# sipposip/pr-disagg-radar-gan

Measured on AMD Instinct MI355X. Metric: cWGAN-GP train samples/sec, 24x16x16 tiles, bs=256, higher is better.
Workload: dtype f32; 1 GPU; ndomain=16, 24h, bs=256 fp32, 1 critic step + 1 gen step (BASELINE configs[1]); batch_per_gpu=256, global_batch=256, n_critic=1, parallelism=dp1, world=1, rccl_ranks_seen=1, weights=random init (RandomNormal 0.02 / glorot_uniform), dropout 0.25 active

## Files before the change

### include/rdgan.h

```cpp
#ifndef RDGAN_H
#define RDGAN_H
#include <stdint.h>
#ifdef __cplusplus
extern "C" {
#endif

typedef struct rdgan_handle rdgan_handle;

#define RDGAN_LATENT_DIM 100
#define RDGAN_NHOURS 24
#define RDGAN_LOSS_SLOTS 8

int rdgan_create(rdgan_handle** out, int ndomain, int n_cond_channels, int max_batch);
void rdgan_destroy(rdgan_handle* h);
const char* rdgan_last_error(const rdgan_handle* h);
long rdgan_gen_param_count(const rdgan_handle* h);
long rdgan_critic_param_count(const rdgan_handle* h);
long rdgan_workspace_bytes(const rdgan_handle* h);

int rdgan_gen_forward(rdgan_handle* h, const float* gen_params, const float* z, const float* cond,
                      float* out, int B, void* stream);

int rdgan_check_numerics(rdgan_handle* h, void* stream);

// ... 128 lines not shown
int rdgan_op_upconv_slab_t16(const float* x, const float* w, const float* bias, float* y, float* rinv, float* dbg, int B, int H, int W,
                             void* stream);
int rdgan_op_upconv2_slab16(const float* x, const float* w, const float* bias, float* y, float* rinv, int B, void* stream);
int rdgan_op_upconv_wgrad_slab16(const float* x, const float* dy, float* dWc, int B, void* stream);
int rdgan_op_d2_fwd_slab16(const float* x, const float* w, const float* bias, float* y, int B, uint64_t seed, void* stream);
int rdgan_op_d2_wgrad_slab16(const float* x, const float* dy, float* dW, int B, void* stream);
int rdgan_op_d2_wgrad_slab_t16(const float* x, const float* dy, float* dW, int B, int OH, int OW, void* stream);
int rdgan_op_d3_wgrad_slab16(const float* x, const float* dy, float* dW, int B, void* stream);
int rdgan_op_d2_dgrad_slab16(const float* gy, const float* w, const float* aux, float* gx, int B, int use_drop, void* stream);
int rdgan_op_d2_dgrad_slab_t16(const float* gy, const float* w, const float* aux, float* gx, int B, int OH, int OW, int use_drop,
                               void* stream);
int rdgan_op_pixelnorm_lrelu(const float* y, float* h, float* rinv, long npix, int C, void* stream);
int rdgan_op_pixelnorm_lrelu_bwd(const float* gh, const float* h, const float* rinv, float* dy,
                                 long npix, int C, void* stream);
int rdgan_debug_activation(rdgan_handle* h, int which, float* out, long n, void* stream);
int rdgan_op_rng(uint64_t seed, uint32_t stream_id, float* mask_out, float* uniform_out, long n,
                 void* stream);

#ifdef __cplusplus
}
#endif
#endif
```

### pr_disagg_radar_gan_amd/_lib.py

```python
import ctypes
import os

_HERE = os.path.dirname(os.path.abspath(__file__))
LIB_PATH = os.path.join(_HERE, "librdgan_hip.so")

c_f32p = ctypes.c_void_p
c_stream = ctypes.c_void_p

class LaunchStat(ctypes.Structure):
    _fields_ = [("plan", ctypes.c_int), ("kind", ctypes.c_int), ("batch", ctypes.c_int), ("launches", ctypes.c_int),
                ("gflop", ctypes.c_double), ("ms", ctypes.c_double), ("name", ctypes.c_char * 48), ("kernel", ctypes.c_char * 48)]


SIGNATURES = {
    "rdgan_create": (ctypes.c_int, [ctypes.POINTER(ctypes.c_void_p), ctypes.c_int, ctypes.c_int, ctypes.c_int]),
    "rdgan_destroy": (None, [ctypes.c_void_p]),
    "rdgan_last_error": (ctypes.c_char_p, [ctypes.c_void_p]),
    "rdgan_gen_param_count": (ctypes.c_long, [ctypes.c_void_p]),
    "rdgan_critic_param_count": (ctypes.c_long, [ctypes.c_void_p]),
    "rdgan_workspace_bytes": (ctypes.c_long, [ctypes.c_void_p]),
    "rdgan_gen_forward": (ctypes.c_int, [ctypes.c_void_p, c_f32p, c_f32p, c_f32p, c_f32p, ctypes.c_int, c_stream]),
    "rdgan_check_numerics": (ctypes.c_int, [ctypes.c_void_p, c_stream]),
    "rdgan_critic_forward": (ctypes.c_int, [ctypes.c_void_p, c_f32p, c_f32p, c_f32p, c_f32p, ctypes.c_int,
                                            ctypes.c_uint64, c_stream]),
# ... 71 lines not shown
    "rdgan_op_fastd_wgrad": (ctypes.c_int, [c_f32p, c_f32p, c_f32p] + [ctypes.c_int] * 8 + [c_stream]),
    "rdgan_op_g9_wgrad": (ctypes.c_int, [c_f32p, c_f32p, c_f32p] + [ctypes.c_int] * 4 + [c_stream]),
    "rdgan_op_upconv_slab16": (ctypes.c_int, [c_f32p] * 6 + [ctypes.c_int, c_stream]),
    "rdgan_op_upconv_slab_t16": (ctypes.c_int, [c_f32p] * 6 + [ctypes.c_int] * 3 + [c_stream]),
    "rdgan_op_upconv2_slab16": (ctypes.c_int, [c_f32p] * 5 + [ctypes.c_int, c_stream]),
    "rdgan_op_upconv_wgrad_slab16": (ctypes.c_int, [c_f32p] * 3 + [ctypes.c_int, c_stream]),
    "rdgan_op_d2_fwd_slab16": (ctypes.c_int, [c_f32p] * 4 + [ctypes.c_int, ctypes.c_uint64, c_stream]),
    "rdgan_op_d3_wgrad_slab16": (ctypes.c_int, [c_f32p] * 3 + [ctypes.c_int, c_stream]),
    "rdgan_op_d2_wgrad_slab16": (ctypes.c_int, [c_f32p] * 3 + [ctypes.c_int, c_stream]),
    "rdgan_op_d2_wgrad_slab_t16": (ctypes.c_int, [c_f32p] * 3 + [ctypes.c_int] * 3 + [c_stream]),
    "rdgan_op_d2_dgrad_slab16": (ctypes.c_int, [c_f32p] * 4 + [ctypes.c_int, ctypes.c_int, c_stream]),
    "rdgan_op_d2_dgrad_slab_t16": (ctypes.c_int, [c_f32p] * 4 + [ctypes.c_int] * 4 + [c_stream]),
    "rdgan_op_pixelnorm_lrelu": (ctypes.c_int, [c_f32p, c_f32p, c_f32p, ctypes.c_long, ctypes.c_int, c_stream]),
    "rdgan_op_pixelnorm_lrelu_bwd": (ctypes.c_int, [c_f32p, c_f32p, c_f32p, c_f32p, ctypes.c_long, ctypes.c_int, c_stream]),
    "rdgan_debug_activation": (ctypes.c_int, [ctypes.c_void_p, ctypes.c_int, c_f32p, ctypes.c_long, c_stream]),
    "rdgan_op_rng": (ctypes.c_int, [ctypes.c_uint64, ctypes.c_uint32, c_f32p, c_f32p, ctypes.c_long, c_stream]),
}

TAG_GCONV_FWD, TAG_GCONV_DGRAD, TAG_GCONV_WGRAD, TAG_CRITIC_GEMM, TAG_ELEMENTWISE, TAG_GCONV3_FWD = range(6)

_lib = None


class RdganError(RuntimeError):
    pass


class NumericsError(RdganError, ArithmeticError):
    """tf.debugging.check_numerics behind the generator's softmax (reference T:349-350) fired: NaN/Inf in the output."""

# ... 27 lines not shown
```

### pr_disagg_radar_gan_amd/csrc/rdgan_api.hip

```cpp
#include <hip/hip_runtime.h>
#include <stdio.h>
#include <string.h>
#include <math.h>
#include <string>
#include <vector>
#include <algorithm>
#include <unordered_set>

#include "../../include/rdgan.h"
#include "rdgan_plan.h"
#include "rdgan_hostplan.h"
#include "rdgan_rng.h"
#include "rdgan_gemm.hip.h"
#include "rdgan_gemm_ws.hip.h"
#include "rdgan_gemm_ws16.hip.h"
#include "rdgan_gemm_f16.hip.h"
#include "rdgan_upconv16.hip.h"
#include "rdgan_upconv16b.hip.h"
#include "rdgan_upconv16t.hip.h"
#include "rdgan_elem.hip.h"
#include "rdgan_data.hip.h"
#include "rdgan_edge.hip.h"
#include "rdgan_d2slab16.hip.h"
#include "rdgan_d2fwd16.hip.h"
// ... 40 lines not shown
  int wgrad_wide = 0;
  int conv_f16 = 1;
  void* bW3I;
  int upconv_slab = 1;
  void* bW3T = nullptr;
  int upconv_slab_t = 1;
  void* bW2I = nullptr;
  int upconv2_slab = 1;
  int g9_fused = 1;
  void* bW9I;
  void* bW2S;
  int d3_wgrad_slab = 1;
  int d2_wgrad_slab = 1;
  int upwgrad_slab = 1;
  int d1_dgrad_fused = 1;
  int d1_wgrad16 = 1;
  void* bW2F = nullptr;
  int d2_fwd_slab = 0;
  unsigned char* g1bits = nullptr;
  int dense16 = 1;
  int dense_skinny = 1;
  void* xcat16 = nullptr;
  void* bW0 = nullptr;
  int g9_bwd_mfma = 1;
  int d1_fwd_sample = 1;
  int wgrad_boxes = 1;
  int border_boxes = 1;
  int d2_gate_bits = 1;
  int d2_slab = 1;
  int a16 = 0;
// ... 622 lines not shown
  const rd_bf16_t* y16 = (const rd_bf16_t*)y; rd_bf16_t* h16 = (rd_bf16_t*)hout;
  if (a16) {
    if (C == 256) hipLaunchKernelGGL((k_pixelnorm_lrelu_fwd<64, rd_bf16_t>), grid, dim3(256), 0, st, y16, h16, rinv, npix);
    else if (C == 128) hipLaunchKernelGGL((k_pixelnorm_lrelu_fwd<32, rd_bf16_t>), grid, dim3(256), 0, st, y16, h16, rinv, npix);
    else if (C == 64) hipLaunchKernelGGL((k_pixelnorm_lrelu_fwd<16, rd_bf16_t>), grid, dim3(256), 0, st, y16, h16, rinv, npix);
    else return bad_arg(h, "pixelnorm: C must be 64/128/256");
  }
  else if (C == 256) hipLaunchKernelGGL(k_pixelnorm_lrelu_fwd<64>, grid, dim3(256), 0, st, y, hout, rinv, npix);
  else if (C == 128) hipLaunchKernelGGL(k_pixelnorm_lrelu_fwd<32>, grid, dim3(256), 0, st, y, hout, rinv, npix);
  else if (C == 64) hipLaunchKernelGGL(k_pixelnorm_lrelu_fwd<16>, grid, dim3(256), 0, st, y, hout, rinv, npix);
  else return bad_arg(h, "pixelnorm: C must be 64/128/256");
  RD_CHECK(h, hipGetLastError());
  return 0;
}
static int launch_pn_bwd(rdgan_handle* h, const float* g, const float* hh, const float* rinv, float* dy, long npix, int C,
                         int pool, int D, int H, int W, hipStream_t st, bool a16 = false) {
  long threads = npix * (C / 4);
  dim3 grid((unsigned)((threads + 255) / 256));
#define RD_PNB(LP, PO) hipLaunchKernelGGL((k_pn_lrelu_bwd<LP, PO>), grid, dim3(256), 0, st, g, hh, rinv, dy, npix, D, H, W)
#define RD_PNB16(LP) hipLaunchKernelGGL((k_pn_lrelu_bwd<LP, 0, rd_bf16_t>), grid, dim3(256), 0, st, (const rd_bf16_t*)g, \
                                        (const rd_bf16_t*)hh, rinv, (rd_bf16_t*)dy, npix, D, H, W)
  if (a16) {
    if (pool) return bad_arg(h, "pixelnorm bwd: the bf16 storage mode needs the collapsed form");
    if (C == 256) RD_PNB16(64); else if (C == 128) RD_PNB16(32); else if (C == 64) RD_PNB16(16);
    else return bad_arg(h, "pixelnorm bwd: C must be 64/128/256");
  }
  else if (C == 256) { if (pool) RD_PNB(64, 1); else RD_PNB(64, 0); }
  else if (C == 128) { if (pool) RD_PNB(32, 1); else RD_PNB(32, 0); }
  else if (C == 64) { if (pool) RD_PNB(16, 1); else RD_PNB(16, 0); }
  else return bad_arg(h, "pixelnorm bwd: C must be 64/128/256");
#undef RD_PNB
#undef RD_PNB16
  RD_CHECK(h, hipGetLastError());
  return 0;
}

static int launch_pn_bwd_pairs(rdgan_handle* h, const float* g, const float* hh, const float* rinv, float* dy, float* gS,
                               long npair, long HW, int C, hipStream_t st, bool a16 = false) {
  long threads = npair * (C / 4);
  dim3 grid((unsigned)((threads + 255) / 256));
#define RD_PNP16(LP) hipLaunchKernelGGL((k_pn_lrelu_bwd_pairs<LP, rd_bf16_t>), grid, dim3(256), 0, st, (const rd_bf16_t*)g, \
                                        (const rd_bf16_t*)hh, rinv, (rd_bf16_t*)dy, (rd_bf16_t*)gS, npair, HW)
  if (a16) {
    if (C == 256) RD_PNP16(64); else if (C == 128) RD_PNP16(32); else if (C == 64) RD_PNP16(16);
    else return bad_arg(h, "pixelnorm bwd: C must be 64/128/256");
  }
  else if (C == 256) hipLaunchKernelGGL(k_pn_lrelu_bwd_pairs<64>, grid, dim3(256), 0, st, g, hh, rinv, dy, gS, npair, HW);
  else if (C == 128) hipLaunchKernelGGL(k_pn_lrelu_bwd_pairs<32>, grid, dim3(256), 0, st, g, hh, rinv, dy, gS, npair, HW);
  else if (C == 64) hipLaunchKernelGGL(k_pn_lrelu_bwd_pairs<16>, grid, dim3(256), 0, st, g, hh, rinv, dy, gS, npair, HW);
  else return bad_arg(h, "pixelnorm bwd: C must be 64/128/256");
#undef RD_PNP16
  RD_CHECK(h, hipGetLastError());
  return 0;
}


extern "C" int rdgan_create(rdgan_handle** out, int ndomain, int n_cond_channels, int max_batch) {
  if (!out) return -2;
  *out = nullptr;
  if (!rd_geometry_ok(ndomain, n_cond_channels, max_batch)) return -2;
  rdgan_handle* h = new rdgan_handle();
  rd_geometry(h, ndomain, n_cond_channels, max_batch);
  const int nd = ndomain;
  const int* gch = h->gch; const int* dch = h->dch;
// ... 195 lines not shown
  if (!strcmp(name, "resident")) { h->resident = value ? 1 : 0; return 0; }
  if (!strcmp(name, "upconv_slab")) { h->upconv_slab = value ? 1 : 0; return 0; }
  if (!strcmp(name, "upconv_slab_t")) { h->upconv_slab_t = value ? 1 : 0; return 0; }
  if (!strcmp(name, "upconv2_slab")) { h->upconv2_slab = value ? 1 : 0; return 0; }
  if (!strcmp(name, "g9_fused")) { h->g9_fused = value ? 1 : 0; return 0; }
  if (!strcmp(name, "d1_fwd_sample")) { h->d1_fwd_sample = value ? 1 : 0; return 0; }
  if (!strcmp(name, "g9_bwd_mfma")) { h->g9_bwd_mfma = value ? 1 : 0; return 0; }
  if (!strcmp(name, "dense16")) { h->dense16 = value ? 1 : 0; return 0; }
  if (!strcmp(name, "dense_skinny")) { h->dense_skinny = value ? 1 : 0; return 0; }
  if (!strcmp(name, "wgrad_boxes")) { h->wgrad_boxes = value ? 1 : 0; return 0; }
  if (!strcmp(name, "border_boxes")) { h->border_boxes = value < 0 ? 0 : (value > 2 ? 2 : value); return 0; }
  if (!strcmp(name, "d3_wgrad_slab")) { h->d3_wgrad_slab = value ? 1 : 0; return 0; }
  if (!strcmp(name, "d2_wgrad_slab")) { h->d2_wgrad_slab = value ? 1 : 0; return 0; }
  if (!strcmp(name, "upwgrad_slab")) { h->upwgrad_slab = value ? 1 : 0; return 0; }
  if (!strcmp(name, "d1_dgrad_fused")) { h->d1_dgrad_fused = value ? 1 : 0; return 0; }
  if (!strcmp(name, "d1_wgrad16")) { h->d1_wgrad16 = value ? 1 : 0; return 0; }
  if (!strcmp(name, "wgrad_wide")) { h->wgrad_wide = value ? 1 : 0; return 0; }
  if (!strcmp(name, "conv_f16")) {
    if (value < 0 || value > 2) return bad_arg(h, "conv_f16: 0, 1 or 2 (2: regardless of the launch size)");
    h->conv_f16 = value; h->ccache_ver = 0; h->gcache_ver = 0; return 0;
  }
  if (!strcmp(name, "d2_fwd_slab")) { h->d2_fwd_slab = value ? 1 : 0; h->ccache_ver = 0; return 0; }
  if (!strcmp(name, "d2_gate_bits")) { h->d2_gate_bits = value ? 1 : 0; return 0; }
  if (!strcmp(name, "d2_slab")) { h->d2_slab = value ? 1 : 0; h->ccache_ver = 0; return 0; }
  if (!strcmp(name, "dense_wgrad_slices")) { h->dense_slices = value; return 0; }
  if (!strcmp(name, "keep_gates")) {
    h->keep_gates = value ? 1 : 0;
    h->gate_keep_B = 0;
    for (int l = 1; l <= 4 && h->keep_gates; ++l)
      if (!h->gate_keep[l]) RD_CHECK(h, hipMalloc(&h->gate_keep[l], (size_t)h->MB * h->dL[l] * h->dch[l] * sizeof(float)));
// ... 655 lines not shown
      const int one = PL_D2B;
      RD_TRY(launch_d2_dgrad_slab_t(h, {one, plan_flops(h->plans[one], NBt), RDGAN_TAG_CRITIC_GEMM}, h->du[2], h->bW2S, h->dh[1], h->du[1], NBt,
                                    h->ddim[2][1], h->ddim[2][2], use_drop, gbits, st));
      continue;
    }
    if (a16)
      RD_TRY(launch_conv16(h, h->plans[pl], h->d_plans + pl, NBt, h->du[l], h->bWB[l], h->du[l - 1], ep, st, RDGAN_TAG_CRITIC_GEMM,
                           h->conv_f16 ? h->fWB[l] : nullptr));
    else
    RD_TRY(launch_conv(h, h->plans[pl], h->d_plans + pl, NBt, h->du[l], h->DWT[l], h->dch[l - 1], h->du[l - 1], ep, st,
                       RDGAN_TAG_CRITIC_GEMM));
  }
  return 0;
}

static int critic_input_grad(rdgan_handle* h, const float* dp, const float* u1, int B, hipStream_t st) {
  if (h->a16 && h->d1_dgrad_fused && h->nd == 16 && d1_gemm_ok(h)) {
    ProfScope ps(h, RDGAN_TAG_CRITIC_GEMM, st);
    LaunchScope ls(h, PL_D1B, RD_KIND_CONV, B, 2.0 * B * h->dL[1] * 27 * 64, st);
    RD_KNAME(h, "k_d1_dgrad_sample16<bf16>");
    h->flops_acc += 2.0 * B * h->dL[1] * 27 * 64;
    RD_TRY(ensure_lds(h, (const void*)k_d1_dgrad_sample16, RD_D1DG_LDS));
    hipLaunchKernelGGL(k_d1_dgrad_sample16, dim3((unsigned)std::min(B, 512)), dim3(256), RD_D1DG_LDS, st, (const rd_bf16_t*)u1,
                       dp + h->doff[0], h->g0, B);
    RD_CHECK(h, hipGetLastError());
    return 0;
  }
  if (h->a16 && h->d1_dgrad_fused && h->nd > 16 && h->nd % 16 == 0 && d1_gemm_ok(h)) {
    ProfScope ps(h, RDGAN_TAG_CRITIC_GEMM, st);
    LaunchScope ls(h, PL_D1B, RD_KIND_CONV, B, 2.0 * B * h->dL[1] * 27 * 64, st);
    RD_KNAME(h, "k_d1_dgrad_tile16<bf16>");
// ... 2 lines not shown
    const long items = (long)B * (h->nd / 16) * (h->nd / 8);
    hipLaunchKernelGGL(k_d1_dgrad_tile16, dim3((unsigned)std::min<long>(items, 1024)), dim3(256), RD_D1DT_LDS, st, (const rd_bf16_t*)u1,
                       dp + h->doff[0], h->g0, B, h->nd);
    RD_CHECK(h, hipGetLastError());
    return 0;
  }
  if (h->a16)
    RD_TRY(launch_conv16(h, h->plans[PL_D1B], h->d_plans + PL_D1B, B, u1, h->bW1B, h->P1, epi_make(RD_EPI_PLAIN), st,
                         RDGAN_TAG_CRITIC_GEMM));
  else
  RD_TRY(launch_conv(h, h->plans[PL_D1B], h->d_plans + PL_D1B, B, u1, h->W1T, h->ldp1, h->P1, epi_make(RD_EPI_PLAIN), st,
                     RDGAN_TAG_CRITIC_GEMM));
  ProfScope ps(h, RDGAN_TAG_ELEMENTWISE, st);
  hipLaunchKernelGGL(k_d1_col2im, dim3(ew_blocks((long)B * h->dL[0])), dim3(256), 0, st, h->P1, h->g0, B, h->ddim[0][0],
                     h->ddim[0][1], h->ddim[0][2], h->ddim[1][0], h->ddim[1][1], h->ddim[1][2], h->Cin, h->ldp1);
  RD_CHECK(h, hipGetLastError());
  return 0;
}

extern "C" int rdgan_critic_forward(rdgan_handle* h, const float* critic_params, const float* sample, const float* cond,
                                    float* out, int B, uint64_t seed, void* stream) {
  if (!h || !critic_params || !sample || !cond || !out) return bad_arg(h, "critic_forward: null pointer");
  if (B < 1 || B > h->NB) return bad_arg(h, "critic_forward: B outside [1, 3*max_batch]");
  hipStream_t st = (hipStream_t)stream;
  RD_TRY(ahead_drain(h, st));
  h->gate_keep_B = 0;
  RD_TRY(a16_check(h));
  if (h->a16) RD_TRY(prep_critic_weights(h, critic_params, st));
  else if (h->CP != h->Cin && !(h->cver_in != 0 && critic_params == h->ccache_ptr && h->cver_in == h->ccache_ver)) {
    hipLaunchKernelGGL(k_pad_w1, dim3(27), dim3(256), 0, st, critic_params + h->doff[0], h->W1P, h->Cin, h->CP);
// ... 36 lines not shown
  const bool a16 = h->a16 != 0;
  {
    ProfScope ps(h, RDGAN_TAG_ELEMENTWISE, st);
    launch_build_critic_input(h, x_real, h->fake, cond, B, 0, rd_make_key(seed, RD_STREAM_ALPHA), (uint32_t)h->sample_offset, st);
  }
  if (gen_z && fwd_ahead_on(h)) RD_TRY(ahead_issue(h, gp, gen_z, gen_cond, gen_B, st));
  RD_TRY(critic_forward_impl(h, dp, NBt, seed, st));
  RD_TRY(critic_dgrad_chain(h, dp, NBt, B, 0, seed, st));
  {
    hipStream_t cs = side_fork(h, st);
    for (int l = 1; l <= 4; ++l) {
      if (l == 1 && d1_gemm_ok(h) && d1_wgrad16_on(h)) continue;
      RD_TRY(launch_colsum(h, h->du[l], (long)2 * B * h->dL[l], h->dch[l], grad + h->doff[2 * (l - 1) + 1], cs, h->a16 != 0));
    }
  }
  RD_TRY(critic_input_grad(h, dp, act_off(h, h->du[1], (long)2 * B * h->dL[1] * 64), B, st));
  float* cin_hat = h->cin + (long)2 * B * h->dL[0] * h->CP;
  {
    ProfScope ps(h, RDGAN_TAG_ELEMENTWISE, st);
    const int per = (int)h->dL[0];
    const int S = std::max(1, std::min({(1024 + B - 1) / B, per / 4096, 64}));
    if (S > 1) hipLaunchKernelGGL(k_gp_norm_part, dim3(B * S), dim3(256), 0, st, h->g0, h->gp_part, per, S);
    hipLaunchKernelGGL(k_gp_norm_r0, dim3(B * S), dim3(256), 0, st, h->g0, cin_hat, h->gpv, per, B, RD_GP_WEIGHT, h->CP, S, h->gp_part);
  }
  h->gate_keep_B = 0;
  if (h->keep_gates) {
    for (int l = 1; l <= 4; ++l) {
      const long third = (long)2 * B * h->dL[l] * h->dch[l];
      RD_CHECK(h, hipMemcpyAsync(h->gate_keep[l], act_off(h, h->dh[l], third), (size_t)(third / 2) * (a16 ? 2 : 4),
                                 hipMemcpyDeviceToDevice, st));
    }
    h->gate_keep_B = B;
  }
  {
    const float* in = cin_hat;
    for (int l = 1; l <= 4; ++l) {
      int pl = l == 1 ? PL_D1F : critic_fwd_plan(h, l, B);
      long third = (long)2 * B * h->dL[l] * h->dch[l];
      float* dst = act_off(h, h->dh[l], third);
// ... 117 lines not shown
    RD_TRY(launch_wgrad(h, h->plans[PL_G9B], h->d_plans + PL_G9B, B, h->P9, h->h3, grad + h->goff[8], h->wpartial,
                        h->wpartial_cap, st, RDGAN_TAG_GCONV_WGRAD));
    RD_TRY(launch_conv(h, h->plans[PL_G9B], h->d_plans + PL_G9B, B, h->P9, gp + h->goff[8], 64, h->gh3,
                       epi_make(RD_EPI_PLAIN), st, RDGAN_TAG_GCONV_DGRAD));
  }
  {
    hipStream_t cs = side_fork(h, st);
    RD_TRY(launch_colsum(h, h->dl, npix3 / 64, 64, h->g9b_tmp, cs));
    RD_TRY(launch_colsum(h, h->g9b_tmp, 64, 1, grad + h->goff[9], cs));
  }
  float* hs[4] = {h->h0, h->h1, h->h2, h->h3};
  float* rs[4] = {nullptr, h->r1, h->r2, h->r3};
  float* dys[4] = {nullptr, h->dy1, h->dy2, h->gh3};
  float* gups[4] = {nullptr, h->gup1, h->gup2, h->gup3};
  const int col = h->collapse;
  if (col) {
    RdSliceMap map;
    collapsed_dgrad_slice_map(map.src);
    for (int l = 1; l <= 3; ++l) {
      if (gen_block_fast(h, l, fast_bwd_on(h))) continue;
      if (gen_block_fast(h, l, fast_fwd_on(h)))
        hipLaunchKernelGGL(k_collapse_weights, dim3(ew_blocks(16L * h->gch[l - 1] * h->gch[l])), dim3(256), 0, st,
                           gp + h->goff[2 * l], h->GWC[l], h->gch[l - 1] * h->gch[l]);
      if (a16) continue;
      hipLaunchKernelGGL(k_transpose_map, dim3((h->gch[l] + 31) / 32, (h->gch[l - 1] + 31) / 32, 64), dim3(256), 0, st,
                         h->GWC[l], h->GWD[l], h->gch[l - 1], h->gch[l], map);
    }
  }
  for (int l = 3; l >= 1; --l) {
    const bool fast = gen_block_fast(h, l, fast_bwd_on(h));
// ... 5 lines not shown
        const int nunits = B * (RDGAN_NHOURS / 2 / PP);
        RD_TRY(ensure_lds(h, (const void*)k_g9_bwd_mfma16, lds9));
        hipLaunchKernelGGL(k_g9_bwd_mfma16, dim3((unsigned)std::min(nunits, PP > 1 ? 768 : 1536)), dim3(256), lds9, st, h->dl, gp + h->goff[8],
                           (const rd_bf16_t*)hs[3], rs[3], (rd_bf16_t*)dys[3], nunits, RDGAN_NHOURS, nd, nd, PP);
      } else
      if (a16) hipLaunchKernelGGL(k_g9_bwd_pairs<rd_bf16_t>, dim3(B * (RDGAN_NHOURS / 2)), dim3(256), g9_lds, st, h->dl, gp + h->goff[8],
                                  (const rd_bf16_t*)hs[3], rs[3], (rd_bf16_t*)dys[3], fast ? (rd_bf16_t*)h->fgS : (rd_bf16_t*)nullptr,
                                  RDGAN_NHOURS, nd, nd);
      else hipLaunchKernelGGL(k_g9_bwd_pairs<float>, dim3(B * (RDGAN_NHOURS / 2)), dim3(256), g9_lds, st, h->dl, gp + h->goff[8],
                              (const float*)hs[3], rs[3], dys[3], fast ? h->fgS : (float*)nullptr, RDGAN_NHOURS, nd, nd);
      RD_CHECK(h, hipGetLastError());
    } else if (fast) {
      ProfScope ps(h, RDGAN_TAG_ELEMENTWISE, st);
      const long HW = (long)h->gdim[l][1] * h->gdim[l][2];
      RD_TRY(launch_pn_bwd_pairs(h, l == 3 ? h->gh3 : gups[l + 1], hs[l], rs[l], dys[l], h->fgS, (long)B * h->gdim[l - 1][0] * HW,
                                 HW, h->gch[l], st, a16));
    } else {
      ProfScope ps(h, RDGAN_TAG_ELEMENTWISE, st);
      if (l == 3) RD_TRY(launch_pn_bwd(h, h->gh3, hs[3], rs[3], dys[3], npix3, 64, 0, 0, 0, 0, st, a16));
      else RD_TRY(launch_pn_bwd(h, gups[l + 1], hs[l], rs[l], dys[l], (long)B * h->gpix[l], h->gch[l], col ? 0 : 1,
                                h->gdim[l][0], h->gdim[l][1], h->gdim[l][2], st, a16));
    }
    const long cc = (long)h->gch[l - 1] * h->gch[l];
    if (fast) {
      const int* sd = h->gdim[l - 1];
      const int D = sd[0];
      const long P = (long)sd[1] * sd[2] * h->gch[l - 1];
      RdWeightMap wm;
      fastd_weight_map(wm);
      {
        ProfScope ps(h, RDGAN_TAG_ELEMENTWISE, st);
        if (!gen_block_fast(h, l, fast_fwd_on(h))) {
          const dim3 dg(ew_blocks((long)B * (D + 1) * P / 4));
          if (a16) hipLaunchKernelGGL(k_diff_d<rd_bf16_t>, dg, dim3(256), 0, st, (const rd_bf16_t*)hs[l - 1], (rd_bf16_t*)h->fE[l], B, D, P);
          else
          hipLaunchKernelGGL(k_diff_d<float>, dg, dim3(256), 0, st, (const float*)hs[l - 1],
                             h->fE[l], B, D, P);
// ... 32 lines not shown
        }
        RD_TRY(launch_conv16(h, h->plans[pbs], h->d_plans + pbs, B, h->fgS, h->bUT, gups[l], eb, st, RDGAN_TAG_GCONV_DGRAD));
        RD_TRY(launch_conv16(h, h->plans[pbe], h->d_plans + pbe, B, dys[l], h->bUT, h->fdE, eb, st, RDGAN_TAG_GCONV_DGRAD));
      } else {
        {
          RdSliceMap map;
          fastd_dgrad_slice_map(map.src);
          hipLaunchKernelGGL(k_transpose_map, dim3((h->gch[l] + 31) / 32, (h->gch[l - 1] + 31) / 32, 48), dim3(256), 0, st, h->fU[l],
                             h->fUT, h->gch[l - 1], h->gch[l], map);
        }
        RD_TRY(launch_conv(h, h->plans[pbs], h->d_plans + pbs, B, h->fgS, h->fUT, h->gch[l - 1], gups[l], eb, st,
                           RDGAN_TAG_GCONV_DGRAD));
        RD_TRY(launch_conv(h, h->plans[pbe], h->d_plans + pbe, B, dys[l], h->fUT, h->gch[l - 1], h->fdE, eb, st,
                           RDGAN_TAG_GCONV_DGRAD));
      }
      {
        ProfScope ps(h, RDGAN_TAG_ELEMENTWISE, st);
        const dim3 cg(ew_blocks((long)B * D * P / 4));
        if (a16) hipLaunchKernelGGL(k_combine_dx<rd_bf16_t>, cg, dim3(256), 0, st, (rd_bf16_t*)gups[l], (const rd_bf16_t*)h->fdE, B, D, P);
        else hipLaunchKernelGGL(k_combine_dx<float>, cg, dim3(256), 0, st, gups[l], (const float*)h->fdE, B, D, P);
      }
    } else if (col) {
      int plf = PL_G1FC + l - 1, plb = gen_box_plan(h, PL_G1BC + l - 1, PL_G1BCX + l - 1, B);
      const int plfx = PL_G1FCX + l - 1;
      const bool wbox = h->wgrad_boxes && h->border_boxes && h->wave_spec && wgrad_box_ok(h->plans[plfx]) &&
                        (h->border_boxes >= 2 || plan_flops(h->plans[plfx], 1) < 0.8 * plan_flops(h->plans[plf], 1));
      bool bias_done = false;
      if (a16 && l == 3 && h->upwgrad_slab && h->nd == 16) {
        RD_TRY(launch_upconv_wgrad_slab(h, {plf, plan_flops(h->plans[plf], B), RDGAN_TAG_GCONV_WGRAD}, hs[l - 1], dys[l], h->wpartial,
                                        h->wpartial_cap, h->dWc, h->ubias_part, grad + h->goff[2 * l + 1], B, st));
        bias_done = true;
// ... 425 lines not shown
  return (int)hipStreamSynchronize(st);
}

extern "C" int rdgan_op_pixelnorm_lrelu(const float* y, float* hout, float* rinv, long npix, int C, void* stream) {
  if (!y || !hout) return -2;
  RD_TRY(launch_pn_fwd(nullptr, y, hout, rinv, npix, C, (hipStream_t)stream));
  return (int)hipStreamSynchronize((hipStream_t)stream);
}
extern "C" int rdgan_op_pixelnorm_lrelu_bwd(const float* gh, const float* hh, const float* rinv, float* dy, long npix, int C,
                                            void* stream) {
  if (!gh || !hh || !rinv || !dy) return -2;
  RD_TRY(launch_pn_bwd(nullptr, gh, hh, rinv, dy, npix, C, 0, 0, 0, 0, (hipStream_t)stream));
  return (int)hipStreamSynchronize((hipStream_t)stream);
}

__global__ void k_bytes_to_f32(const unsigned char* in, float* out, long n) {
  for (long i = blockIdx.x * (long)blockDim.x + threadIdx.x; i < n; i += (long)gridDim.x * blockDim.x) out[i] = (float)in[i];
}
extern "C" int rdgan_debug_activation(rdgan_handle* h, int which, float* out, long n, void* stream) {
  if (h) RD_TRY(ahead_drain(h, (hipStream_t)stream));
  if (h && out && which == 8 && n >= 1) {
    if (!h->g1bits || n > (long)h->NB * h->dL[1] * 16) return bad_arg(h, "debug_activation: no gate bytes");
    hipLaunchKernelGGL(k_bytes_to_f32, dim3(ew_blocks(n)), dim3(256), 0, (hipStream_t)stream, h->g1bits, out, n);
    RD_CHECK(h, hipGetLastError());
    return 0;
  }
  if (!h || !out || which < 0 || which > 7 || n < 1) return bad_arg(h, "debug_activation: bad argument");
  const float* src; long cap;
  if (which < 4) {
    float* hs[4] = {h->h0, h->h1, h->h2, h->h3};
// ... 482 lines not shown
```

### pr_disagg_radar_gan_amd/csrc/rdgan_edge.hip.h

```cpp
#pragma once
#include "rdgan_gemm_ws16.hip.h"

template <typename T>
__global__ void __launch_bounds__(256, 2)
k_g9_fwd(const T* __restrict__ h3, const float* __restrict__ w9 , float* __restrict__ Q, long rows, int Wd,
         int HW, int NQ) {
  constexpr bool BF = sizeof(T) == 2;
  constexpr int ROWB = BF ? 128 : 256;
  constexpr int CST = 33;
  extern __shared__ __attribute__((aligned(16))) float smem[];
  float* As = smem;
  float* Ws = smem + 256 * ROWB / 4;
  const int tid = threadIdx.x, lane = tid & 63;
  const int wave = __builtin_amdgcn_readfirstlane(tid >> 6);
  const int l31 = lane & 31, lhalf = lane >> 5;
  const long m0 = (long)blockIdx.x * 256;

  {
    const __amdgpu_buffer_rsrc_t rs = rd_make_rsrc((const float*)(h3 + m0 * 64));
    constexpr int RPI = 1024 / ROWB;
    constexpr int CPR = ROWB / 16;
#pragma unroll
    for (int k = 0; k < 64 / RPI; ++k) {
      const int r = wave * 64 + k * RPI + lane / CPR;
// ... 634 lines not shown
          const u32x4_t z = {0u, 0u, 0u, 0u};
          acc = __builtin_amdgcn_mfma_f32_32x32x16_bf16(__builtin_bit_cast(rd_bf16x8, ok ? a[i][kk] : z), wf[kk], acc, 0, 0, 0);
        }
#pragma unroll
        for (int r = 0; r < 16; ++r) Dl[(blk * 32 + (r & 3) + 8 * (r >> 2) + 4 * lhalf) * 33 + l31] = acc[r];
      }
    }
    __syncthreads();
    float* gb = g0 + (long)b * 6144;
    rd_d1dg_class<0, 0, 0>(Dl, gb, tid); rd_d1dg_class<0, 0, 1>(Dl, gb, tid); rd_d1dg_class<0, 1, 0>(Dl, gb, tid);
    rd_d1dg_class<0, 1, 1>(Dl, gb, tid); rd_d1dg_class<1, 0, 0>(Dl, gb, tid); rd_d1dg_class<1, 0, 1>(Dl, gb, tid);
    rd_d1dg_class<1, 1, 0>(Dl, gb, tid); rd_d1dg_class<1, 1, 1>(Dl, gb, tid);
    __syncthreads();
  }
}

#define RD_D1DT_LDS (512 * 33 * 4)
template <int PD, int PH, int PW>
__device__ __forceinline__ void rd_d1dt_class(const float* __restrict__ Dl, float* __restrict__ gb, int tid, int nd, int O, int oh0, int ow0,
                                              int h0, int w0) {
#pragma unroll
  for (int it = 0; it < 2; ++it) {
    const int i = tid + it * 256;
    if (i >= 384) break;
    const int dq = i >> 5, hq = (i >> 2) & 7, wq = i & 3;
    float sum = 0.f;
#pragma unroll
    for (int jd = 0; jd < (PD ? 1 : 2); ++jd) {
      const int td = PD ? 1 : 2 * jd, od = PD ? dq : dq - jd;
      const bool vd = od >= 0 && od < 11;
// ... 310 lines not shown
```

### pr_disagg_radar_gan_amd/csrc/rdgan_elem.hip.h

```cpp
#pragma once
#include <hip/hip_runtime.h>
#include "rdgan_gemm.hip.h"

#define RD_PIXELNORM_EPS 1.0e-8f

__device__ __forceinline__ float rd_wave_sum(float v) {
#pragma unroll
  for (int o = 32; o > 0; o >>= 1) v += __shfl_xor(v, o, 64);
  return v;
}
template <int LP>
__device__ __forceinline__ float rd_seg_sum(float v) {
#pragma unroll
  for (int o = LP / 2; o > 0; o >>= 1) v += __shfl_xor(v, o, 64);
  return v;
}
__device__ __forceinline__ void rd_store_bf16x4(unsigned short* p, f32x4 v) { rd_st4(p, v); }
__device__ __forceinline__ float rd_block_sum(float v, float* red) {
  v = rd_wave_sum(v);
  if ((threadIdx.x & 63) == 0) red[threadIdx.x >> 6] = v;
  __syncthreads();
  float s = 0.f;
  if (threadIdx.x == 0)
    for (int i = 0; i < (int)(blockDim.x >> 6); ++i) s += red[i];
// ... 43 lines not shown
  n.y = hv.y > 0.f ? hv.y : hv.y * (1.0f / RD_LRELU_ALPHA);
  n.z = hv.z > 0.f ? hv.z : hv.z * (1.0f / RD_LRELU_ALPHA);
  n.w = hv.w > 0.f ? hv.w : hv.w * (1.0f / RD_LRELU_ALPHA);
  gn.x = gh.x * rd_lrelu_slope_from_out(hv.x);
  gn.y = gh.y * rd_lrelu_slope_from_out(hv.y);
  gn.z = gh.z * rd_lrelu_slope_from_out(hv.z);
  gn.w = gh.w * rd_lrelu_slope_from_out(hv.w);
  const float dot = rd_seg_sum<LP>(gn.x * n.x + gn.y * n.y + gn.z * n.z + gn.w * n.w) * (1.0f / C);
  f32x4 o;
  o.x = ri * (gn.x - n.x * dot); o.y = ri * (gn.y - n.y * dot);
  o.z = ri * (gn.z - n.z * dot); o.w = ri * (gn.w - n.w * dot);
  return o;
}
template <int LP, int POOL, typename T = float>
__global__ void k_pn_lrelu_bwd(const T* __restrict__ g, const T* __restrict__ h, const float* __restrict__ rinv,
                               T* __restrict__ dy, long npix, int D, int H, int W) {
  constexpr int C = LP * 4;
  const long gid = blockIdx.x * (long)blockDim.x + threadIdx.x;
  const long pix = gid / LP;
  const int sub = (int)(gid % LP);
  const bool ok = pix < npix;
  f32x4 gh = {0.f, 0.f, 0.f, 0.f}, hv = {0.f, 0.f, 0.f, 0.f};
  float ri = 0.f;
  if (ok) {
    hv = rd_ld4(h + pix * C + sub * 4);
    ri = rinv[pix];
    if (POOL) {
      long t = pix;
      int w = (int)(t % W); t /= W;
      int hh = (int)(t % H); t /= H;
      int d = (int)(t % D);
      long b = t / D;
#pragma unroll
      for (int e = 0; e < 8; ++e) {
        long up = (((b * (2 * D) + 2 * d + (e >> 2)) * (2 * H) + 2 * hh + ((e >> 1) & 1)) * (2 * W) + 2 * w + (e & 1));
        gh += rd_ld4(g + up * C + sub * 4);
      }
    } else {
      gh = rd_ld4(g + pix * C + sub * 4);
    }
  }
  const f32x4 o = rd_pn_lrelu_bwd_row<LP>(gh, hv, ri);
  if (ok) rd_st4(dy + pix * C + sub * 4, o);
}
template <int LP, typename T = float>
__global__ void k_pn_lrelu_bwd_pairs(const T* __restrict__ g, const T* __restrict__ h, const float* __restrict__ rinv,
                                     T* __restrict__ dy, T* __restrict__ gS, long npair, long HW) {
  constexpr int C = LP * 4;
  const long gid = blockIdx.x * (long)blockDim.x + threadIdx.x;
  const long pr = gid / LP;
  const int sub = (int)(gid % LP);
  const bool ok = pr < npair;
  const long bs = pr / HW, hw = pr - bs * HW;
  const long pixA = (2 * bs) * HW + hw, pixB = pixA + HW;
  f32x4 ga = {0.f, 0.f, 0.f, 0.f}, ha = ga, gb = ga, hb = ga;
  float ra = 0.f, rb = 0.f;
  if (ok) {
    ga = rd_ld4(g + pixA * C + sub * 4); ha = rd_ld4(h + pixA * C + sub * 4); ra = rinv[pixA];
    gb = rd_ld4(g + pixB * C + sub * 4); hb = rd_ld4(h + pixB * C + sub * 4); rb = rinv[pixB];
  }
  const f32x4 oa = rd_pn_lrelu_bwd_row<LP>(ga, ha, ra);
  const f32x4 ob = rd_pn_lrelu_bwd_row<LP>(gb, hb, rb);
  if (ok) {
    rd_st4(dy + pixA * C + sub * 4, oa);
    rd_st4(dy + pixB * C + sub * 4, ob);
    rd_st4(gS + pr * C + sub * 4, oa + ob);
  }
}

template <typename T = float>
__global__ void __launch_bounds__(256)
k_g9_bwd_pairs(const float* __restrict__ dl, const float* __restrict__ w9, const T* __restrict__ h3,
               const float* __restrict__ rinv, T* __restrict__ dy, T* __restrict__ gS, int D, int H, int W) {
  extern __shared__ __attribute__((aligned(16))) float dls[];
// ... 874 lines not shown
```

### pr_disagg_radar_gan_amd/engine.py

```python
import ctypes
import itertools

import numpy as np
import torch

from . import _lib
from . import weights as W

LOSS_SLOTS = 8

_versions = itertools.count(1)


def new_version():
    return next(_versions)


def require_gpu():
    if not torch.cuda.is_available():
        raise _lib.RdganError("no MI355X/ROCm device visible: the cWGAN-GP hot path runs only on the HIP "
                              "library (there is deliberately no CPU fallback)")


def _ptr(t):
# ... 159 lines not shown
        _lib.check(self.lib.rdgan_adam(_ptr(params), _ptr(grad), _ptr(v), n, int(t), float(lr), float(beta2), float(eps),
                                       float(grad_scale), self._stream()), self._h, "rdgan_adam")

    def set_option(self, name, value):
        _lib.check(self.lib.rdgan_set_option(self._h, name.encode(), int(value)), self._h, "rdgan_set_option")

    def profile(self, tag_mask):
        _lib.check(self.lib.rdgan_profile(self._h, int(tag_mask)), self._h, "rdgan_profile")

    def debug_activation(self, which, shape):
        out = torch.empty(tuple(shape), dtype=torch.float32, device=self.device)
        _lib.check(self.lib.rdgan_debug_activation(self._h, int(which), _ptr(out), out.numel(), self._stream()), self._h,
                   "rdgan_debug_activation")
        return out

    def flop_count(self, reset=False):
        f = ctypes.c_double()
        _lib.check(self.lib.rdgan_flop_count(self._h, ctypes.byref(f), int(bool(reset))), self._h, "rdgan_flop_count")
        return f.value

    def profile_launches(self, on):
        _lib.check(self.lib.rdgan_profile_launches(self._h, int(bool(on))), self._h, "rdgan_profile_launches")

    def launch_table(self):
        buf = (_lib.LaunchStat * 256)()
        n = ctypes.c_int()
        _lib.check(self.lib.rdgan_launch_table(self._h, buf, 256, ctypes.byref(n)), self._h, "rdgan_launch_table")
        kinds = {0: "gemm", 1: "wgrad", 2: "edge"}
        return [dict(name=r.name.decode(), kernel=r.kernel.decode(), kind=kinds.get(r.kind, "?"), batch=r.batch,
                     launches=r.launches, gflop=r.gflop, ms=r.ms) for r in buf[:n.value]]
# ... 7 lines not shown
```

Measured before the change: 23930 samples/s.

## Fuse critic input-grad with GP norm and fold combine_dx into pixelnorm backward

Adds an fp32 MFMA kernel for the critic's first-layer input gradient. An optional GP mode of that kernel also computes the per-sample gradient norm, the penalty value and the scaled cin_hat in the same pass, replacing the separate norm kernels. Separately, the generator backward skips the standalone k_combine_dx pass for upper layers and instead adds the dE difference inside the pixelnorm/lrelu backward kernels. This cuts launches and global-memory round trips, at the cost of a heavier single-occupancy kernel with extra LDS. It also adds a debug entry point for checking the fused input gradient.

```diff
diff --git a/include/rdgan.h b/include/rdgan.h
--- a/include/rdgan.h
+++ b/include/rdgan.h
@@ -166,6 +166,8 @@
 int rdgan_op_pixelnorm_lrelu_bwd(const float* gh, const float* h, const float* rinv, float* dy,
                                  long npix, int C, void* stream);
 int rdgan_debug_activation(rdgan_handle* h, int which, float* out, long n, void* stream);
+int rdgan_debug_d1_input_grad(rdgan_handle* h, const float* critic_params, const float* u1, int B, int with_norm,
+                              float* g0_out, float* cin_hat_out, float* gp_out, void* stream);
 int rdgan_op_rng(uint64_t seed, uint32_t stream_id, float* mask_out, float* uniform_out, long n,
                  void* stream);
 
diff --git a/pr_disagg_radar_gan_amd/_lib.py b/pr_disagg_radar_gan_amd/_lib.py
--- a/pr_disagg_radar_gan_amd/_lib.py
+++ b/pr_disagg_radar_gan_amd/_lib.py
@@ -109,6 +109,8 @@
     "rdgan_op_pixelnorm_lrelu": (ctypes.c_int, [c_f32p, c_f32p, c_f32p, ctypes.c_long, ctypes.c_int, c_stream]),
     "rdgan_op_pixelnorm_lrelu_bwd": (ctypes.c_int, [c_f32p, c_f32p, c_f32p, c_f32p, ctypes.c_long, ctypes.c_int, c_stream]),
     "rdgan_debug_activation": (ctypes.c_int, [ctypes.c_void_p, ctypes.c_int, c_f32p, ctypes.c_long, c_stream]),
+    "rdgan_debug_d1_input_grad": (ctypes.c_int, [ctypes.c_void_p, c_f32p, c_f32p, ctypes.c_int, ctypes.c_int, c_f32p, c_f32p, c_f32p,
+                                                 c_stream]),
     "rdgan_op_rng": (ctypes.c_int, [ctypes.c_uint64, ctypes.c_uint32, c_f32p, c_f32p, ctypes.c_long, c_stream]),
 }
 
diff --git a/pr_disagg_radar_gan_amd/csrc/rdgan_api.hip b/pr_disagg_radar_gan_amd/csrc/rdgan_api.hip
--- a/pr_disagg_radar_gan_amd/csrc/rdgan_api.hip
+++ b/pr_disagg_radar_gan_amd/csrc/rdgan_api.hip
@@ -78,6 +78,7 @@
   int d2_wgrad_slab = 1;
   int upwgrad_slab = 1;
   int d1_dgrad_fused = 1;
+  int combine_dx_fused = 1;
   int d1_wgrad16 = 1;
   void* bW2F = nullptr;
   int d2_fwd_slab = 0;
@@ -730,12 +731,13 @@
   return 0;
 }
 static int launch_pn_bwd(rdgan_handle* h, const float* g, const float* hh, const float* rinv, float* dy, long npix, int C,
-                         int pool, int D, int H, int W, hipStream_t st, bool a16 = false) {
+                         int pool, int D, int H, int W, hipStream_t st, bool a16 = false, const float* dE = nullptr) {
   long threads = npix * (C / 4);
   dim3 grid((unsigned)((threads + 255) / 256));
-#define RD_PNB(LP, PO) hipLaunchKernelGGL((k_pn_lrelu_bwd<LP, PO>), grid, dim3(256), 0, st, g, hh, rinv, dy, npix, D, H, W)
+  if (dE && (a16 || pool || D < 1 || H < 1 || W < 1)) return bad_arg(h, "pixelnorm bwd: dE needs fp32 storage and the collapsed form");
+#define RD_PNB(LP, PO) hipLaunchKernelGGL((k_pn_lrelu_bwd<LP, PO>), grid, dim3(256), 0, st, g, hh, rinv, dy, npix, D, H, W, dE)
 #define RD_PNB16(LP) hipLaunchKernelGGL((k_pn_lrelu_bwd<LP, 0, rd_bf16_t>), grid, dim3(256), 0, st, (const rd_bf16_t*)g, \
-                                        (const rd_bf16_t*)hh, rinv, (rd_bf16_t*)dy, npix, D, H, W)
+                                        (const rd_bf16_t*)hh, rinv, (rd_bf16_t*)dy, npix, D, H, W, (const rd_bf16_t*)nullptr)
   if (a16) {
     if (pool) return bad_arg(h, "pixelnorm bwd: the bf16 storage mode needs the collapsed form");
     if (C == 256) RD_PNB16(64); else if (C == 128) RD_PNB16(32); else if (C == 64) RD_PNB16(16);
@@ -752,18 +754,19 @@
 }
 
 static int launch_pn_bwd_pairs(rdgan_handle* h, const float* g, const float* hh, const float* rinv, float* dy, float* gS,
-                               long npair, long HW, int C, hipStream_t st, bool a16 = false) {
+                               long npair, long HW, int C, hipStream_t st, bool a16 = false, const float* dE = nullptr, int Ds = 1) {
   long threads = npair * (C / 4);
   dim3 grid((unsigned)((threads + 255) / 256));
+  if (dE && (a16 || Ds < 1)) return bad_arg(h, "pixelnorm bwd: dE needs fp32 storage");
 #define RD_PNP16(LP) hipLaunchKernelGGL((k_pn_lrelu_bwd_pairs<LP, rd_bf16_t>), grid, dim3(256), 0, st, (const rd_bf16_t*)g, \
-                                        (const rd_bf16_t*)hh, rinv, (rd_bf16_t*)dy, (rd_bf16_t*)gS, npair, HW)
+                                        (const rd_bf16_t*)hh, rinv, (rd_bf16_t*)dy, (rd_bf16_t*)gS, npair, HW, (const rd_bf16_t*)nullptr, 1)
   if (a16) {
     if (C == 256) RD_PNP16(64); else if (C == 128) RD_PNP16(32); else if (C == 64) RD_PNP16(16);
     else return bad_arg(h, "pixelnorm bwd: C must be 64/128/256");
   }
-  else if (C == 256) hipLaunchKernelGGL(k_pn_lrelu_bwd_pairs<64>, grid, dim3(256), 0, st, g, hh, rinv, dy, gS, npair, HW);
-  else if (C == 128) hipLaunchKernelGGL(k_pn_lrelu_bwd_pairs<32>, grid, dim3(256), 0, st, g, hh, rinv, dy, gS, npair, HW);
-  else if (C == 64) hipLaunchKernelGGL(k_pn_lrelu_bwd_pairs<16>, grid, dim3(256), 0, st, g, hh, rinv, dy, gS, npair, HW);
+  else if (C == 256) hipLaunchKernelGGL(k_pn_lrelu_bwd_pairs<64>, grid, dim3(256), 0, st, g, hh, rinv, dy, gS, npair, HW, dE, Ds);
+  else if (C == 128) hipLaunchKernelGGL(k_pn_lrelu_bwd_pairs<32>, grid, dim3(256), 0, st, g, hh, rinv, dy, gS, npair, HW, dE, Ds);
+  else if (C == 64) hipLaunchKernelGGL(k_pn_lrelu_bwd_pairs<16>, grid, dim3(256), 0, st, g, hh, rinv, dy, gS, npair, HW, dE, Ds);
   else return bad_arg(h, "pixelnorm bwd: C must be 64/128/256");
 #undef RD_PNP16
   RD_CHECK(h, hipGetLastError());
@@ -989,6 +992,7 @@
   if (!strcmp(name, "d2_wgrad_slab")) { h->d2_wgrad_slab = value ? 1 : 0; return 0; }
   if (!strcmp(name, "upwgrad_slab")) { h->upwgrad_slab = value ? 1 : 0; return 0; }
   if (!strcmp(name, "d1_dgrad_fused")) { h->d1_dgrad_fused = value ? 1 : 0; return 0; }
+  if (!strcmp(name, "combine_dx_fused")) { h->combine_dx_fused = value ? 1 : 0; return 0; }
   if (!strcmp(name, "d1_wgrad16")) { h->d1_wgrad16 = value ? 1 : 0; return 0; }
   if (!strcmp(name, "wgrad_wide")) { h->wgrad_wide = value ? 1 : 0; return 0; }
   if (!strcmp(name, "conv_f16")) {
@@ -1674,7 +1678,29 @@
   return 0;
 }
 
-static int critic_input_grad(rdgan_handle* h, const float* dp, const float* u1, int B, hipStream_t st) {
+static int critic_input_grad(rdgan_handle* h, const float* dp, const float* u1, int B, hipStream_t st, float* cin_hat = nullptr,
+                             bool* norm_done = nullptr) {
+  if (norm_done) *norm_done = false;
+  if (!h->a16 && h->d1_dgrad_fused && h->nd == 16 && d1_gemm_ok(h)) {
+    ProfScope ps(h, RDGAN_TAG_CRITIC_GEMM, st);
+    LaunchScope ls(h, PL_D1B, RD_KIND_CONV, B, 2.0 * B * h->dL[1] * 27 * 64, st);
+    h->flops_acc += 2.0 * B * h->dL[1] * 27 * 64;
+    const dim3 grid((unsigned)std::min(B, 512));
+    if (cin_hat && norm_done) {
+      RD_KNAME(h, "k_d1_dgrad_sample32<gp>");
+      RD_TRY(ensure_lds(h, (const void*)k_d1_dgrad_sample32<true>, RD_D1DG_LDS_GP));
+      hipLaunchKernelGGL(k_d1_dgrad_sample32<true>, grid, dim3(256), RD_D1DG_LDS_GP, st, u1, dp + h->doff[0], h->g0, B, cin_hat, h->gpv,
+                         RD_GP_WEIGHT);
+      *norm_done = true;
+    } else {
+      RD_KNAME(h, "k_d1_dgrad_sample32");
+      RD_TRY(ensure_lds(h, (const void*)k_d1_dgrad_sample32<false>, RD_D1DG_LDS));
+      hipLaunchKernelGGL(k_d1_dgrad_sample32<false>, grid, dim3(256), RD_D1DG_LDS, st, u1, dp + h->doff[0], h->g0, B, (float*)nullptr,
+                         (float*)nullptr, 0.f);
+    }
+    RD_CHECK(h, hipGetLastError());
+    return 0;
+  }
   if (h->a16 && h->d1_dgrad_fused && h->nd == 16 && d1_gemm_ok(h)) {
     ProfScope ps(h, RDGAN_TAG_CRITIC_GEMM, st);
     LaunchScope ls(h, PL_D1B, RD_KIND_CONV, B, 2.0 * B * h->dL[1] * 27 * 64, st);
@@ -1707,6 +1733,19 @@
   ProfScope ps(h, RDGAN_TAG_ELEMENTWISE, st);
   hipLaunchKernelGGL(k_d1_col2im, dim3(ew_blocks((long)B * h->dL[0])), dim3(256), 0, st, h->P1, h->g0, B, h->ddim[0][0],
                      h->ddim[0][1], h->ddim[0][2], h->ddim[1][0], h->ddim[1][1], h->ddim[1][2], h->Cin, h->ldp1);
+  RD_CHECK(h, hipGetLastError());
+  return 0;
+}
+
+static int critic_penalty_input(rdgan_handle* h, const float* dp, const float* u1, int B, float* cin_hat, hipStream_t st) {
+  bool norm_done = false;
+  RD_TRY(critic_input_grad(h, dp, u1, B, st, cin_hat, &norm_done));
+  if (norm_done) return 0;
+  ProfScope ps(h, RDGAN_TAG_ELEMENTWISE, st);
+  const int per = (int)h->dL[0];
+  const int S = std::max(1, std::min({(1024 + B - 1) / B, per / 4096, 64}));
+  if (S > 1) hipLaunchKernelGGL(k_gp_norm_part, dim3(B * S), dim3(256), 0, st, h->g0, h->gp_part, per, S);
+  hipLaunchKernelGGL(k_gp_norm_r0, dim3(B * S), dim3(256), 0, st, h->g0, cin_hat, h->gpv, per, B, RD_GP_WEIGHT, h->CP, S, h->gp_part);
   RD_CHECK(h, hipGetLastError());
   return 0;
 }
@@ -1773,15 +1812,8 @@
       RD_TRY(launch_colsum(h, h->du[l], (long)2 * B * h->dL[l], h->dch[l], grad + h->doff[2 * (l - 1) + 1], cs, h->a16 != 0));
     }
   }
-  RD_TRY(critic_input_grad(h, dp, act_off(h, h->du[1], (long)2 * B * h->dL[1] * 64), B, st));
   float* cin_hat = h->cin + (long)2 * B * h->dL[0] * h->CP;
-  {
-    ProfScope ps(h, RDGAN_TAG_ELEMENTWISE, st);
-    const int per = (int)h->dL[0];
-    const int S = std::max(1, std::min({(1024 + B - 1) / B, per / 4096, 64}));
-    if (S > 1) hipLaunchKernelGGL(k_gp_norm_part, dim3(B * S), dim3(256), 0, st, h->g0, h->gp_part, per, S);
-    hipLaunchKernelGGL(k_gp_norm_r0, dim3(B * S), dim3(256), 0, st, h->g0, cin_hat, h->gpv, per, B, RD_GP_WEIGHT, h->CP, S, h->gp_part);
-  }
+  RD_TRY(critic_penalty_input(h, dp, act_off(h, h->du[1], (long)2 * B * h->dL[1] * 64), B, cin_hat, st));
   h->gate_keep_B = 0;
   if (h->keep_gates) {
     for (int l = 1; l <= 4; ++l) {
@@ -1929,6 +1961,7 @@
   float* dys[4] = {nullptr, h->dy1, h->dy2, h->gh3};
   float* gups[4] = {nullptr, h->gup1, h->gup2, h->gup3};
   const int col = h->collapse;
+  const float* dE_in = nullptr;
   if (col) {
     RdSliceMap map;
     collapsed_dgrad_slice_map(map.src);
@@ -1964,13 +1997,14 @@
       ProfScope ps(h, RDGAN_TAG_ELEMENTWISE, st);
       const long HW = (long)h->gdim[l][1] * h->gdim[l][2];
       RD_TRY(launch_pn_bwd_pairs(h, l == 3 ? h->gh3 : gups[l + 1], hs[l], rs[l], dys[l], h->fgS, (long)B * h->gdim[l - 1][0] * HW,
-                                 HW, h->gch[l], st, a16));
+                                 HW, h->gch[l], st, a16, l == 3 ? nullptr : dE_in, h->gdim[l - 1][0]));
     } else {
       ProfScope ps(h, RDGAN_TAG_ELEMENTWISE, st);
       if (l == 3) RD_TRY(launch_pn_bwd(h, h->gh3, hs[3], rs[3], dys[3], npix3, 64, 0, 0, 0, 0, st, a16));
       else RD_TRY(launch_pn_bwd(h, gups[l + 1], hs[l], rs[l], dys[l], (long)B * h->gpix[l], h->gch[l], col ? 0 : 1,
-                                h->gdim[l][0], h->gdim[l][1], h->gdim[l][2], st, a16));
-    }
+                                h->gdim[l][0], h->gdim[l][1], h->gdim[l][2], st, a16, dE_in));
+    }
+    dE_in = nullptr;
     const long cc = (long)h->gch[l - 1] * h->gch[l];
     if (fast) {
       const int* sd = h->gdim[l - 1];
@@ -2033,7 +2067,8 @@
         RD_TRY(launch_conv(h, h->plans[pbe], h->d_plans + pbe, B, dys[l], h->fUT, h->gch[l - 1], h->fdE, eb, st,
                            RDGAN_TAG_GCONV_DGRAD));
       }
-      {
+      if (!a16 && h->combine_dx_fused && l >= 2) dE_in = h->fdE;
+      else {
         ProfScope ps(h, RDGAN_TAG_ELEMENTWISE, st);
         const dim3 cg(ew_blocks((long)B * D * P / 4));
         if (a16) hipLaunchKernelGGL(k_combine_dx<rd_bf16_t>, cg, dim3(256), 0, st, (rd_bf16_t*)gups[l], (const rd_bf16_t*)h->fdE, B, D, P);
@@ -2489,6 +2524,25 @@
   return (int)hipStreamSynchronize((hipStream_t)stream);
 }
 
+extern "C" int rdgan_debug_d1_input_grad(rdgan_handle* h, const float* critic_params, const float* u1, int B, int with_norm,
+                                         float* g0_out, float* cin_hat_out, float* gp_out, void* stream) {
+  if (!h || !critic_params || !u1 || !g0_out) return bad_arg(h, "debug_d1_input_grad: null pointer");
+  if (with_norm && (!cin_hat_out || !gp_out)) return bad_arg(h, "debug_d1_input_grad: with_norm needs cin_hat_out and gp_out");
+  if (B < 1 || B > h->MB) return bad_arg(h, "debug_d1_input_grad: B outside [1, max_batch]");
+  if (h->a16) return bad_arg(h, "debug_d1_input_grad: fp32 storage only");
+  hipStream_t st = (hipStream_t)stream;
+  RD_TRY(ahead_drain(h, st));
+  RD_TRY(prep_critic_weights(h, critic_params, st));
+  if (with_norm) {
+    RD_TRY(critic_penalty_input(h, critic_params, u1, B, h->cin, st));
+    RD_CHECK(h, hipMemcpyAsync(cin_hat_out, h->cin, sizeof(float) * B * h->dL[0] * h->CP, hipMemcpyDeviceToDevice, st));
+    RD_CHECK(h, hipMemcpyAsync(gp_out, h->gpv, sizeof(float) * B, hipMemcpyDeviceToDevice, st));
+  } else
+    RD_TRY(critic_input_grad(h, critic_params, u1, B, st));
+  RD_CHECK(h, hipMemcpyAsync(g0_out, h->g0, sizeof(float) * B * h->dL[0], hipMemcpyDeviceToDevice, st));
+  return 0;
+}
+
 __global__ void k_bytes_to_f32(const unsigned char* in, float* out, long n) {
   for (long i = blockIdx.x * (long)blockDim.x + threadIdx.x; i < n; i += (long)gridDim.x * blockDim.x) out[i] = (float)in[i];
 }
diff --git a/pr_disagg_radar_gan_amd/csrc/rdgan_edge.hip.h b/pr_disagg_radar_gan_amd/csrc/rdgan_edge.hip.h
--- a/pr_disagg_radar_gan_amd/csrc/rdgan_edge.hip.h
+++ b/pr_disagg_radar_gan_amd/csrc/rdgan_edge.hip.h
@@ -672,6 +672,74 @@
     __syncthreads();
   }
 }
+#define RD_D1DG_LDS_GP (RD_D1DG_LDS + 6144 * 4)
+template <bool GP>
+__global__ void __launch_bounds__(256, GP ? 1 : 2)
+k_d1_dgrad_sample32(const float* __restrict__ u1, const float* __restrict__ w1, float* __restrict__ g0, int B,
+                    float* __restrict__ cin_hat, float* __restrict__ gp_out, float gp_weight) {
+  extern __shared__ __attribute__((aligned(16))) float Dl[];
+  __shared__ float red[4];
+  __shared__ float coef_s;
+  const int tid = threadIdx.x, lane = tid & 63;
+  const int wave = __builtin_amdgcn_readfirstlane(tid >> 6);
+  const int l31 = lane & 31, lhalf = lane >> 5;
+  f32x4 wf[8];
+#pragma unroll
+  for (int j = 0; j < 8; ++j) {
+    const f32x4 z = {0.f, 0.f, 0.f, 0.f};
+    wf[j] = l31 < 27 ? *(const f32x4*)(w1 + (l31 * 2) * 64 + (j * 2 + lhalf) * 4) : z;
+  }
+  for (int b = blockIdx.x; b < B; b += gridDim.x) {
+    const float* ub = u1 + (long)b * (539 * 64);
+    f32x4 a[5][8];
+#pragma unroll
+    for (int i = 0; i < 5; ++i) {
+      const int row = (wave + 4 * i) * 32 + l31;
+      const float* rp = ub + (long)(row < 539 ? row : 0) * 64 + lhalf * 4;
+#pragma unroll
+      for (int j = 0; j < 8; ++j) a[i][j] = *(const f32x4*)(rp + j * 8);
+    }
+#pragma unroll
+    for (int i = 0; i < 5; ++i) {
+      const int blk = wave + 4 * i;
+      if (blk < 17) {
+        const bool ok = blk * 32 + l31 < 539;
+        f32x16 acc;
+#pragma unroll
+        for (int r = 0; r < 16; ++r) acc[r] = 0.f;
+#pragma unroll
+        for (int j = 0; j < 8; ++j)
+#pragma unroll
+          for (int s = 0; s < 4; ++s)
+            acc = __builtin_amdgcn_mfma_f32_32x32x2f32(ok ? a[i][j][s] : 0.f, wf[j][s], acc, 0, 0, 0);
+#pragma unroll
+        for (int r = 0; r < 16; ++r) Dl[(blk * 32 + (r & 3) + 8 * (r >> 2) + 4 * lhalf) * 33 + l31] = acc[r];
+      }
+    }
+    __syncthreads();
+    float* gg = g0 + (long)b * 6144;
+    float* gb = GP ? Dl + 544 * 33 : gg;
+    rd_d1dg_class<0, 0, 0>(Dl, gb, tid); rd_d1dg_class<0, 0, 1>(Dl, gb, tid); rd_d1dg_class<0, 1, 0>(Dl, gb, tid);
+    rd_d1dg_class<0, 1, 1>(Dl, gb, tid); rd_d1dg_class<1, 0, 0>(Dl, gb, tid); rd_d1dg_class<1, 0, 1>(Dl, gb, tid);
+    rd_d1dg_class<1, 1, 0>(Dl, gb, tid); rd_d1dg_class<1, 1, 1>(Dl, gb, tid);
+    __syncthreads();
+    if (GP) {
+      float s = 0.f;
+      for (int i = tid; i < 6144; i += 256) { const float v = gb[i]; gg[i] = v; s += v * v; }
+      s = rd_block_sum(s, red);
+      if (tid == 0) {
+        const float n = sqrtf(s);
+        gp_out[b] = n - 1.0f;
+        coef_s = (gp_weight / B) * 2.0f * (n - 1.0f) / n;
+      }
+      __syncthreads();
+      const float coef = coef_s;
+      float2* o = (float2*)cin_hat + (long)b * 6144;
+      for (int i = tid; i < 6144; i += 256) { const float2 v = {coef * gb[i], 0.f}; o[i] = v; }
+      __syncthreads();
+    }
+  }
+}
 
 #define RD_D1DT_LDS (512 * 33 * 4)
 template <int PD, int PH, int PW>
diff --git a/pr_disagg_radar_gan_amd/csrc/rdgan_elem.hip.h b/pr_disagg_radar_gan_amd/csrc/rdgan_elem.hip.h
--- a/pr_disagg_radar_gan_amd/csrc/rdgan_elem.hip.h
+++ b/pr_disagg_radar_gan_amd/csrc/rdgan_elem.hip.h
@@ -81,7 +81,7 @@
 }
 template <int LP, int POOL, typename T = float>
 __global__ void k_pn_lrelu_bwd(const T* __restrict__ g, const T* __restrict__ h, const float* __restrict__ rinv,
-                               T* __restrict__ dy, long npix, int D, int H, int W) {
+                               T* __restrict__ dy, long npix, int D, int H, int W, const T* __restrict__ dE = nullptr) {
   constexpr int C = LP * 4;
   const long gid = blockIdx.x * (long)blockDim.x + threadIdx.x;
   const long pix = gid / LP;
@@ -105,6 +105,11 @@
       }
     } else {
       gh = rd_ld4(g + pix * C + sub * 4);
+      if (dE) {
+        const long HW = (long)H * W, bd = pix / HW, b = bd / D;
+        const T* e = dE + ((bd + b) * HW + (pix - bd * HW)) * C + sub * 4;
+        gh += rd_ld4(e) - rd_ld4(e + HW * C);
+      }
     }
   }
   const f32x4 o = rd_pn_lrelu_bwd_row<LP>(gh, hv, ri);
@@ -112,7 +117,8 @@
 }
 template <int LP, typename T = float>
 __global__ void k_pn_lrelu_bwd_pairs(const T* __restrict__ g, const T* __restrict__ h, const float* __restrict__ rinv,
-                                     T* __restrict__ dy, T* __restrict__ gS, long npair, long HW) {
+                                     T* __restrict__ dy, T* __restrict__ gS, long npair, long HW,
+                                     const T* __restrict__ dE = nullptr, int Ds = 1) {
   constexpr int C = LP * 4;
   const long gid = blockIdx.x * (long)blockDim.x + threadIdx.x;
   const long pr = gid / LP;
@@ -125,6 +131,12 @@
   if (ok) {
     ga = rd_ld4(g + pixA * C + sub * 4); ha = rd_ld4(h + pixA * C + sub * 4); ra = rinv[pixA];
     gb = rd_ld4(g + pixB * C + sub * 4); hb = rd_ld4(h + pixB * C + sub * 4); rb = rinv[pixB];
+    if (dE) {
+      const T* e = dE + ((2 * bs + bs / Ds) * HW + hw) * C + sub * 4;
+      const f32x4 e0 = rd_ld4(e), e1 = rd_ld4(e + HW * C), e2 = rd_ld4(e + 2 * HW * C);
+      ga += e0 - e1;
+      gb += e1 - e2;
+    }
   }
   const f32x4 oa = rd_pn_lrelu_bwd_row<LP>(ga, ha, ra);
   const f32x4 ob = rd_pn_lrelu_bwd_row<LP>(gb, hb, rb);
diff --git a/pr_disagg_radar_gan_amd/engine.py b/pr_disagg_radar_gan_amd/engine.py
--- a/pr_disagg_radar_gan_amd/engine.py
+++ b/pr_disagg_radar_gan_amd/engine.py
@@ -197,6 +197,20 @@
                    "rdgan_debug_activation")
         return out
 
+    def debug_d1_input_grad(self, critic_params, u1, with_norm=False):
+        B, nd = u1.shape[0], self.ndomain
+        self._check_batch(B, self.max_batch)
+        _chk_tensor(critic_params, (self.n_critic,), "critic_params")
+        _chk_tensor(u1, (B, u1.shape[1], 64), "u1")
+        g0 = torch.empty((B, W.NHOURS, nd, nd), dtype=torch.float32, device=self.device)
+        cin_hat = torch.empty((B, W.NHOURS * nd * nd, 1 + self.n_cond_channels), dtype=torch.float32, device=self.device) if with_norm else None
+        gp = torch.empty((B,), dtype=torch.float32, device=self.device) if with_norm else None
+        _lib.check(self.lib.rdgan_debug_d1_input_grad(self._h, _ptr(critic_params), _ptr(u1), B, int(bool(with_norm)), _ptr(g0),
+                                                      ctypes.c_void_p(cin_hat.data_ptr() if with_norm else 0),
+                                                      ctypes.c_void_p(gp.data_ptr() if with_norm else 0), self._stream()),
+                   self._h, "rdgan_debug_d1_input_grad")
+        return (g0, cin_hat, gp) if with_norm else g0
+
     def flop_count(self, reset=False):
         f = ctypes.c_double()
         _lib.check(self.lib.rdgan_flop_count(self._h, ctypes.byref(f), int(bool(reset))), self._h, "rdgan_flop_count")
```

New measurement: 24220 samples/s (median of 6 runs). 1.01x the previous value.
